# nchopin/particles

Measured on NVIDIA H100. Metric: particle-steps/sec (N x T), Bootstrap SV, higher is better.
Workload: dtype f64

## Files before the change

### particles_b200/csrc/smcb_filter.cu

```cuda
#include <stdlib.h>

#include "smcb_step.cuh"

extern template int bind_fk<GordonM>(smcb_filter *);
extern template int bind_fk<ThetaLogisticM>(smcb_filter *);
extern template int bind_fk<DiscreteCoxM>(smcb_filter *);
extern template int bind_fk<StochVolLevM>(smcb_filter *);
extern template int bind_fk<BearingsM>(smcb_filter *);
extern template int bind_fk<MvLinGaussM<2>>(smcb_filter *);
extern template int bind_fk<MvLinGaussM<3>>(smcb_filter *);
extern template int bind_fk<MvLinGaussM<4>>(smcb_filter *);

static int filter_bind(smcb_filter *f) {
    const smcb_filter_desc *d = &f->desc;
    bool bound = false;
    const int rc = with_model(d->model, d->dim, [&](auto m) {
        using M = decltype(m);
        if (M::D != d->dim) return SMCB_ENOSYS;
        bound = true;
        return bind_fk<M>(f);
    });
    if (bound) return rc;
    if (d->dim != 1 && d->model == SMCB_MODEL_BEARINGS) {
        set_error("fused BearingsOnly: state dimension must be 4");
        return SMCB_EINVAL;
    }
    if (d->dim == 1) set_error("fused filter: model id %d is not available in the fused 1-D family", d->model);
    else if (d->model == SMCB_MODEL_MVLINGAUSS) set_error("fused MVLinearGauss: dx must be 2, 3 or 4 (got %d)", d->dim);
    else set_error("fused filter: model id %d has no d-dimensional kernel", d->model);
    return SMCB_ENOSYS;
}

static int filter_setup(smcb_filter *f, smcb_ctx *c, const smcb_filter_desc *d);

extern "C" int smcb_filter_create(smcb_ctx *c, const smcb_filter_desc *d, smcb_filter **out) {
    SMCB_REQUIRE(c && d && out, "smcb_filter_create: NULL argument");
    SMCB_REQUIRE(d->n >= 1 && d->T >= 1, "smcb_filter_create: need n >= 1 and T >= 1");
    SMCB_REQUIRE(d->X[0] && d->X[1] && d->lw[0] && d->lw[1] && d->A && d->cdf && d->data && d->summaries,
                 "smcb_filter_create: NULL device buffer");
    SMCB_REQUIRE((d->index_offset & 1) == 0, "smcb_filter_create: index_offset must be even");
    SMCB_REQUIRE(d->dim >= 1 && d->dim <= 4, "smcb_filter_create: fused kernels exist for state dimension 1..4 (dim=%d)", d->dim);
    SMCB_REQUIRE(d->dy >= 1 && d->dy <= kMaxDy, "smcb_filter_create: observation dimension must be 1..%d", kMaxDy);
    SMCB_REQUIRE(d->essrmin >= 0.0 && d->essrmin <= 1.0, "smcb_filter_create: ESSrmin must be in [0, 1]");
    smcb_filter *f = new (std::nothrow) smcb_filter();
    SMCB_REQUIRE(f != nullptr, "smcb_filter_create: out of host memory");
    f->ctx = c;
    f->desc = *d;
    f->t_host = 0;
    f->timed = false;
    f->mem = nullptr;
    const int rc = filter_setup(f, c, d);
    if (rc) {
        if (f->mem) cudaFree(f->mem);
        delete f;
        return rc;
    }
    *out = f;
    return SMCB_OK;
}

static bool env_flag(const char *name, bool dflt) {
    const char *v = getenv(name);
    if (!v || !*v) return dflt;
    return v[0] != '0';
}

static int filter_setup(smcb_filter *f, smcb_ctx *c, const smcb_filter_desc *d) {
    int rc = filter_bind(f);
    if (rc) return rc;

    const int64_t n = d->n;
    FilterArgs &a = f->args;
    memset(&a, 0, sizeof(a));
    a.math_tab = c->math_tab;
    a.X[0] = d->X[0]; a.X[1] = d->X[1]; a.lw[0] = d->lw[0]; a.lw[1] = d->lw[1];
    a.A = reinterpret_cast<long long *>(d->A);
    a.cdf = d->cdf;
    a.su = (d->scheme == SMCB_RS_MULTINOMIAL) ? d->scratch : nullptr;
    SMCB_REQUIRE(d->scheme != SMCB_RS_MULTINOMIAL || d->scratch != nullptr,
                 "smcb_filter_create: multinomial needs desc.scratch of n + 2 doubles");
    a.data = d->data;
    a.sc = d->step_consts;
    a.summaries = d->summaries;
    a.moments = d->moments;
    a.z_in = d->z_in; a.u_in = d->u_in;
    a.dy = d->dy;
    a.n = n; a.n_global = d->n_global > 0 ? d->n_global : n;
    a.index_offset = d->index_offset; a.T = d->T;
    a.essrmin = d->essrmin;
    a.key = key_of(d->seed);
    {
        int dev = 0, sms = kSMs;
        SMCB_CUDA(cudaGetDevice(&dev));
        SMCB_CUDA(cudaDeviceGetAttribute(&sms, cudaDevAttrMultiProcessorCount, dev));
        const int64_t npairs = (n + 1) / 2;
        int64_t g = sms < kMaxStepGrid ? sms : kMaxStepGrid;
        const int64_t gmax = (npairs + f->block_size - 1) / f->block_size;
        if (g > gmax) g = gmax;
        if (g < 1) g = 1;
        int64_t chunk = (npairs + g - 1) / g;
        g = (npairs + chunk - 1) / chunk;
        a.chunk = chunk;
        f->grid_move = (int)g;
        a.grid = f->grid_move;
        const bool apf = d->fk == SMCB_FK_APF || d->fk == SMCB_FK_AUXBOOT;
        const bool mom = d->moments != nullptr;
        a.slab_lane = (!apf && !mom) ? 1 : 0;
        a.slab_stride = a.slab_lane ? 96 : 4 + (apf ? 4 : 0) + (mom ? 2 * d->dim : 0);
        const int64_t cap = f->slab_doubles / a.slab_stride;
        const int64_t n_iter = (chunk + f->pairs_per_iteration - 1) / f->pairs_per_iteration;
        int64_t slab_it = 2, n_small = 0;
        for (;; slab_it++) {
            const int64_t ns = (cap * slab_it - n_iter) / (slab_it - 1) - 1;
            const int64_t want = n_iter < 32 ? n_iter : 32;
            if (ns >= want) { n_small = ns < 0 ? 0 : (ns > n_iter / 8 ? n_iter / 8 : ns); break; }
        }
        if (n_small > n_iter) n_small = n_iter;
        a.slab_it = (int)slab_it;
        a.slab_small = (int)n_small;
    }
    a.world = d->world > 1 ? d->world : 1;
    a.rank = d->world > 1 ? d->rank : 0;
    {
        const char *v = getenv("SMCB_FUSE");
        const int mode = (!v || !*v) ? 1 : (v[0] == '0' ? 0 : (v[0] == '2' ? 2 : 1));
        a.fuse_mode = (d->dim == 1 && a.world == 1) ? mode : 0;
    }
    constexpr size_t kHdr = 512;
    static_assert(2 * sizeof(StepState) <= 256, "StepState outgrew its header slot");
    const size_t part = (size_t)kPartSlots * kMaxStepGrid * kPartStride * sizeof(double);
    const size_t agg = (size_t)(kMaxStepGrid + 8) * sizeof(double);
    const size_t slab = a.fuse_mode ? (size_t)f->grid_move * f->slab_doubles * sizeof(double) : 0;
    SMCB_CUDA(cudaMalloc(&f->mem, kHdr + part + agg + slab));
    SMCB_CUDA(cudaMemsetAsync(f->mem, 0, kHdr + part + agg, c->stream));
    a.st = reinterpret_cast<StepState *>(f->mem);
    a.fuse = reinterpret_cast<long long *>(f->mem + 256);
    a.bar = reinterpret_cast<unsigned long long *>(f->mem + 384);
    a.sync_timeout = reinterpret_cast<int *>(f->mem + 392);
    a.partials = reinterpret_cast<double *>(f->mem + kHdr);
    a.blk_agg = reinterpret_cast<double *>(f->mem + kHdr + part);
    a.fuse_slab = a.fuse_mode ? reinterpret_cast<double *>(f->mem + kHdr + part + agg) : nullptr;
    a.local_stats = d->local_stats;
    a.gathered = d->gathered;
    a.mail_local = (a.world > 1) ? d->mail_local : nullptr;
    for (int r = 0; r < 8; r++) a.mail_peer[r] = (a.world > 1 && r < a.world) ? d->mail_peer[r] : nullptr;
    SMCB_REQUIRE(a.world == 1 || (a.rank >= 0 && a.rank < a.world), "smcb_filter_create: bad rank");
    SMCB_REQUIRE(a.world == 1 || a.mail_local || (d->local_stats && d->gathered),
                 "smcb_filter_create: world > 1 needs either a peer mailbox or local_stats / gathered");
    SMCB_REQUIRE(a.world <= 8, "smcb_filter_create: at most 8 ranks");
    if (a.mail_local) {
        for (int r = 0; r < a.world; r++)
            SMCB_REQUIRE(a.mail_peer[r] != nullptr, "smcb_filter_create: mail_peer[%d] is NULL", r);
    }
    a.rs_global = (a.world > 1 && d->rs_global) ? 1 : 0;
    if (a.rs_global) {
        SMCB_REQUIRE(a.mail_local != nullptr, "smcb_filter_create: global resampling needs the peer mailbox");
        SMCB_REQUIRE((n & 1) == 0, "smcb_filter_create: global resampling needs an even shard size");
        if (d->scheme != SMCB_RS_SYSTEMATIC && d->scheme != SMCB_RS_STRATIFIED) {
            set_error("fused filter: global resampling over shards supports systematic and stratified");
            return SMCB_ENOSYS;
        }
        for (int r = 0; r < a.world; r++) {
            SMCB_REQUIRE(d->peer_X0[r] && d->peer_X1[r] && d->peer_cdf[r],
                         "smcb_filter_create: peer_X0 / peer_X1 / peer_cdf[%d] is NULL", r);
            a.pX[r][0] = d->peer_X0[r]; a.pX[r][1] = d->peer_X1[r]; a.pcdf[r] = d->peer_cdf[r];
        }
    }
    f->pdl = env_flag("SMCB_PDL", true);
    f->coop = env_flag("SMCB_COOP", false);
    return SMCB_OK;
}

extern "C" int smcb_filter_destroy(smcb_filter *f) {
    if (!f) return SMCB_OK;
    cudaStreamSynchronize(f->ctx->stream);
    cudaFree(f->mem);
    delete f;
    return SMCB_OK;
}

static int launch_one(smcb_filter *f) {
    if (f->t_host >= f->desc.T) {
        set_error("smcb_filter_step: all %lld steps already done (StopIteration)", (long long)f->desc.T);
        return SMCB_EINVAL;
    }
    int rc = (f->t_host == 0) ? f->launch_init(f) : f->launch_step(f);
    if (rc && f->t_host > 0 && (f->pdl || f->coop)) {
        cudaGetLastError();
        f->pdl = false; f->coop = false;
        rc = f->launch_step(f);
    }
    if (rc) return rc;
    f->t_host++;
    return SMCB_OK;
}

extern "C" int smcb_filter_step_local(smcb_filter *f) {
    SMCB_REQUIRE(f != nullptr && f->args.world > 1 && f->args.mail_local == nullptr,
                 "smcb_filter_step_local: not a sharded filter with the host-driven exchange");
    f->args.batch_end = f->t_host + 1;
    int rc = launch_one(f);
    if (rc) return rc;
    return f->launch_publish(f);
}

extern "C" int smcb_filter_step_finish(smcb_filter *f) {
    SMCB_REQUIRE(f != nullptr && f->args.world > 1, "smcb_filter_step_finish: not a sharded filter");
    return f->launch_tail(f);
}

extern "C" int smcb_filter_step(smcb_filter *f, int64_t nsteps) {
    SMCB_REQUIRE(f != nullptr, "smcb_filter_step: NULL filter");
    SMCB_REQUIRE(f->args.world == 1 || f->args.mail_local != nullptr,
                 "smcb_filter_step: sharded filters without a peer mailbox use step_local / step_finish");
    if (nsteps <= 0) return SMCB_OK;
    f->args.batch_end = f->t_host + nsteps;
    for (int64_t i = 0; i < nsteps; i++) {
        int rc = launch_one(f);
        if (rc) return rc;
    }
    return f->launch_tail(f);
}

extern "C" int smcb_filter_step_timed(smcb_filter *f, int64_t nsteps, double *out8) {
    SMCB_REQUIRE(f && out8, "smcb_filter_step_timed: NULL argument");
    SMCB_REQUIRE(nsteps >= 1 && nsteps <= 100000, "smcb_filter_step_timed: nsteps out of range");
    SMCB_REQUIRE(f->t_host + nsteps <= f->desc.T, "smcb_filter_step_timed: past the last step");
    SMCB_REQUIRE(f->args.world == 1, "smcb_filter_step_timed: single-device filters only");
    cudaStream_t s = f->ctx->stream;
    const size_t nev = (size_t)(nsteps + 1) * 2;
    cudaEvent_t *ev = new (std::nothrow) cudaEvent_t[nev];
    double *rows = new (std::nothrow) double[(size_t)nsteps * SMCB_SUMMARY_STRIDE];
    size_t made = 0;
    int rc = SMCB_OK;
    const int64_t t_first = f->t_host;
    auto fail = [&](cudaError_t e, const char *what) {
        set_error("smcb_filter_step_timed: %s -> %s", what, cudaGetErrorString(e));
        rc = SMCB_ECUDA;
    };
    if (!ev || !rows) { set_error("smcb_filter_step_timed: out of host memory"); rc = SMCB_EINVAL; }
    for (; rc == SMCB_OK && made < nev; made++) {
        cudaError_t e = cudaEventCreate(&ev[made]);
        if (e != cudaSuccess) { fail(e, "cudaEventCreate"); break; }
    }
    f->timed = true;
    f->args.batch_end = t_first + nsteps;
    for (int64_t i = 0; rc == SMCB_OK && i <= nsteps; i++) {
        cudaEventRecord(ev[2 * i], s);
        rc = (i < nsteps) ? launch_one(f) : f->launch_tail(f);
        cudaEventRecord(ev[2 * i + 1], s);
    }
    f->timed = false;
    if (rc == SMCB_OK) {
        cudaError_t e = cudaStreamSynchronize(s);
        if (e != cudaSuccess) fail(e, "cudaStreamSynchronize");
    }
    if (rc == SMCB_OK) {
        cudaError_t e = cudaMemcpy(rows, f->args.summaries + (size_t)t_first * SMCB_SUMMARY_STRIDE,
                                   sizeof(double) * nsteps * SMCB_SUMMARY_STRIDE, cudaMemcpyDeviceToHost);
        if (e != cudaSuccess) fail(e, "cudaMemcpy(summaries)");
    }
    if (rc == SMCB_OK) {
        for (int j = 0; j < 8; j++) out8[j] = 0.0;
        for (int64_t i = 0; i <= nsteps; i++) {
            float ms = 0.f;
            cudaEventElapsedTime(&ms, ev[2 * i], ev[2 * i + 1]);
            int kind = 2;
            if (i < nsteps) {
                const int64_t t = t_first + i;
                kind = (t == 0) ? 0 : (rows[(size_t)i * SMCB_SUMMARY_STRIDE + 2] != 0.0 ? 1 : 3);
            }
            out8[kind] += ms;
            out8[4 + kind] += 1.0;
        }
    }
    for (size_t i = 0; i < made; i++) cudaEventDestroy(ev[i]);
    delete[] ev;
    delete[] rows;
    return rc;
}
// ... 65 lines not shown
```

### particles_b200/csrc/smcb_step.cuh

```cuda
#pragma once
#include <string.h>

#include <new>
#include <type_traits>

#include "smcb_common.cuh"
#include "smcb_dispatch.cuh"
#include "smcb_math.cuh"
#include "smcb_models.cuh"
#include "smcb_scan.cuh"
#include "smcb_search.cuh"

using namespace smcb;

namespace smcb {

constexpr int kPartStride = 16;
constexpr int kMailStride = 32;
constexpr int kMailEpoch = 16;
constexpr int kMailScan = 17;
constexpr int kMaxStepGrid = 256;
constexpr int kMaxD = 4;
constexpr int kTailBlock = 256;
constexpr int kPartSlots = 4;
#ifndef SMCB_SPECULATE
#define SMCB_SPECULATE 1
#endif
template <class M> struct StepCfg {
    static constexpr int BS = 512;
    static constexpr int kU = (M::D == 1) ? 2 : 1;
    static constexpr int kStage = 8 * BS;
    static constexpr int kSlabRecords = 128;
    static constexpr int kSlabDoubles = kSlabRecords * 96;
    static constexpr size_t dyn_smem = kMathTabBytes + (size_t)(2 * kStage > kSlabDoubles ? 2 * kStage : kSlabDoubles) * sizeof(double);
};
constexpr int kScanGroupWarps = 2;
constexpr int kMovePairs = 2;

struct StepState {
    double logLt, log_mean_w, ess;
    double wm, ws, wq;
    long long t;
    long long nrs;
    int rs;
    int rs_next;
    int pad[2];
};

struct FilterArgs {
    double *X[2];
    double *lw[2];
    long long *A;
    double *cdf;
    double *su;
    const double *data;
    const double *sc;
    double *summaries;
    double *moments;
    const double *z_in, *u_in;
    StepState *st;
    int *sync_timeout;
    double *partials;
    int fuse_mode;
    int64_t batch_end;
    long long *fuse;
    double *fuse_slab;
    unsigned long long *bar;
    double *blk_agg;
    const double *math_tab;
    int slab_it;
    int slab_small;
    int slab_lane;
    int slab_stride;
    int64_t n, n_global, index_offset, T;
    int dy;
    int world, rank;
    int grid;
    int64_t chunk;
    double essrmin;
    Philox key;
    double *local_stats;
    const double *gathered;
    double *mail_local;
    double *mail_peer[8];
    int rs_global;
    const double *pX[8][2];
    const double *pcdf[8];
};

__device__ __forceinline__ void wait_epoch(const volatile double *flag, double epoch, int *timeout) {
    const long long t0 = clock64();
    if (*reinterpret_cast<volatile int *>(timeout)) return;
    while (*flag < epoch) {
        if (clock64() - t0 > 8000000000ll) { *timeout = 1; break; }
    }
    __threadfence_system();
}

__device__ __forceinline__ StepK step_consts(const FilterArgs &a, long long t) {
    StepK k;
    k.t = t;
#pragma unroll
    for (int i = 0; i < kMaxDy; i++) {
        k.yv[i] = (i < a.dy && t >= 0) ? a.data[t * a.dy + i] : 0.0;
        k.yn[i] = (i < a.dy && t + 1 < a.T) ? a.data[(t + 1) * a.dy + i] : 0.0;
    }
    k.y = k.yv[0];
    k.y_next = k.yn[0];
    k.sc0 = (a.sc && t >= 0) ? a.sc[t] : 0.0;
    return k;
}

__device__ __forceinline__ double fix_nan(double v) { return v != v ? -CUDART_INF : v; }

__device__ __forceinline__ void weights_scalars(const Lse3 &a, double n, double &log_mean, double &ess) {
    if (a.m == -CUDART_INF || a.m == CUDART_INF || a.m != a.m) {
        log_mean = CUDART_NAN;
        ess = CUDART_NAN;
        return;
    }
    log_mean = a.m + log(a.s / n);
    ess = (a.s * a.s) / a.q;
}

__device__ __forceinline__ double shift_factor(double m, double M) {
    return (m == -CUDART_INF) ? 0.0 : fexp_neg(m - M);
}

__device__ __forceinline__ double nanmax(double a, double b) { return (b > a || b != b) ? b : a; }

template <int NV, int BS, bool MAX>
__device__ __forceinline__ void block_reduce_all(double (&v)[NV], double *smem) {
    constexpr int NWARP = BS / 32;
    static_assert(NWARP <= 32, "one lane per warp in the second level");
    const int lane = threadIdx.x & 31, warp = threadIdx.x >> 5;
#pragma unroll
    for (int j = 0; j < NV; j++) {
#pragma unroll
        for (int mask = 16; mask > 0; mask >>= 1) {
            const double o = __shfl_xor_sync(0xffffffffu, v[j], mask);
            v[j] = MAX ? nanmax(v[j], o) : v[j] + o;
        }
    }
    if (lane == 0) {
#pragma unroll
        for (int j = 0; j < NV; j++) smem[warp * NV + j] = v[j];
    }
    __syncthreads();
    if (warp == 0) {
#pragma unroll
        for (int j = 0; j < NV; j++) {
            double x = (lane < NWARP) ? smem[lane * NV + j] : (MAX ? -CUDART_INF : 0.0);
#pragma unroll
            for (int mask = 16; mask > 0; mask >>= 1) {
                const double o = __shfl_xor_sync(0xffffffffu, x, mask);
                x = MAX ? nanmax(x, o) : x + o;
            }
            if (lane == 0) smem[NWARP * NV + j] = x;
        }
    }
    __syncthreads();
#pragma unroll
    for (int j = 0; j < NV; j++) v[j] = smem[NWARP * NV + j];
    __syncthreads();
}
template <int NV, int BS>
__device__ __forceinline__ void block_max_all(double (&v)[NV], double *smem) { block_reduce_all<NV, BS, true>(v, smem); }
template <int NV, int BS>
__device__ __forceinline__ void block_sum_all(double (&v)[NV], double *smem) { block_reduce_all<NV, BS, false>(v, smem); }

template <int D>
struct Acc {
    Lse3 w;
    double sx[D], sxx[D];
};

template <int D>
__device__ __forceinline__ void acc_init(Acc<D> &a) {
    a.w = lse3_empty();
#pragma unroll
    for (int c = 0; c < D; c++) { a.sx[c] = 0.0; a.sxx[c] = 0.0; }
}

template <int NV, int D, bool FINITE, bool MOM>
__device__ __forceinline__ void acc_add_batch_t(Acc<D> &a, const double (&v)[NV], const double (&x)[NV][D]) {
    double mb = v[0];
#pragma unroll
    for (int j = 1; j < NV; j++) mb = FINITE ? (v[j] > mb ? v[j] : mb) : fmax(mb, v[j]);
    if (mb > a.w.m) {
        const double r = texp_neg(a.w.m - mb);
        a.w.s *= r;
        a.w.q *= r * r;
        if (MOM) {
#pragma unroll
            for (int c = 0; c < D; c++) { a.sx[c] *= r; a.sxx[c] *= r; }
        }
        a.w.m = mb;
    }
    if (!FINITE && a.w.m == -CUDART_INF) return;
#pragma unroll
    for (int j = 0; j < NV; j++) {
        const double e = FINITE ? texp_sat(v[j] - a.w.m) : texp_neg(v[j] - a.w.m);
        a.w.s += e;
        a.w.q = fma(e, e, a.w.q);
        if (MOM && (FINITE || v[j] != -CUDART_INF)) {
#pragma unroll
            for (int c = 0; c < D; c++) {
                const double ex = e * x[j][c];
                a.sx[c] += ex;
                a.sxx[c] = fma(ex, x[j][c], a.sxx[c]);
            }
        }
    }
}
template <int NV, int D, bool FINITE = false>
__device__ __forceinline__ void acc_add_batch(Acc<D> &a, const double (&v)[NV], const double (&x)[NV][D], bool mom) {
    if (mom) acc_add_batch_t<NV, D, FINITE, true>(a, v, x);
    else acc_add_batch_t<NV, D, FINITE, false>(a, v, x);
}

struct StepSmem {
    double red[32 * 16];
    int next;
    double ringP[32];
    int ringF[32];
    double gwarp[16][8];
    double gpref[16][2];
    int gqn[16];
    long long gq[16][8][3];
    int *timeout_ptr;
    double peer[8][kMailStride];
    double goff[9], gpi[8];
    double pref[2];
    double carry[20];
};

__device__ __forceinline__ double shift_factor_t(double m, double M) {
    return (m == -CUDART_INF) ? 0.0 : texp_neg(m - M);
}

__device__ __forceinline__ double warp_max_nan(double v) {
#pragma unroll
    for (int mask = 16; mask > 0; mask >>= 1) {
        const double o = __shfl_xor_sync(0xffffffffu, v, mask);
        v = (o > v || o != o) ? o : v;
    }
    return v;
}
__device__ __forceinline__ double warp_sum(double v) {
#pragma unroll
    for (int mask = 16; mask > 0; mask >>= 1) v += __shfl_xor_sync(0xffffffffu, v, mask);
    return v;
}

template <int D, bool APF>
__device__ __forceinline__ void warp_reduce_to_slab(const Acc<D> &sa, const Lse3 &sx, bool mom, double *rec, int lane) {
    const double M = warp_max_nan(sa.w.m);
    const double e = shift_factor_t(sa.w.m, M);
    const double s = warp_sum(sa.w.s * e), q = warp_sum(sa.w.q * (e * e));
    if (lane == 0) { rec[0] = M; rec[1] = s; rec[2] = q; }
    int off = 4;
    if (APF) {
        const double Ma = warp_max_nan(sx.m);
        const double ea = shift_factor_t(sx.m, Ma);
        const double as_ = warp_sum(sx.s * ea), aq = warp_sum(sx.q * (ea * ea));
        if (lane == 0) { rec[4] = Ma; rec[5] = as_; rec[6] = aq; }
        off = 8;
    }
    if (mom) {
#pragma unroll
        for (int c = 0; c < D; c++) {
            const double a1 = warp_sum(sa.sx[c] * e), a2 = warp_sum(sa.sxx[c] * e);
            if (lane == 0) { rec[off + c] = a1; rec[off + D + c] = a2; }
        }
    }
}

template <int D, bool APF, int BS>
__device__ __forceinline__ void write_partial(const FilterArgs &a, long long t, const Acc<D> &acc, const Lse3 &aux,
                                              bool mom, StepSmem &sh, const double *s_slab = nullptr, int n_slab = 0) {
    const bool lane_rec = a.slab_lane != 0;
    const int n_rec = lane_rec ? n_slab * 32 : n_slab;
    auto rec_ptr = [&](int r) {
        return lane_rec ? s_slab + (size_t)(r >> 5) * a.slab_stride + (r & 31) : s_slab + (size_t)r * a.slab_stride;
    };
    const int rs_ = lane_rec ? 32 : 1;
    if (n_slab > 0) __syncthreads();
    double mx[2] = {acc.w.m, APF ? aux.m : -CUDART_INF};
    for (int r = threadIdx.x; r < n_rec; r += BS) {
        const double *rec = rec_ptr(r);
        mx[0] = nanmax(mx[0], rec[0]);
        if (APF && !lane_rec) mx[1] = nanmax(mx[1], rec[4]);
    }
    block_max_all<2, BS>(mx, sh.red);
    const double ew = shift_factor_t(acc.w.m, mx[0]);
    const double ea = APF ? shift_factor_t(aux.m, mx[1]) : 0.0;
    double v[4 + 2 * D];
    v[0] = acc.w.s * ew;
    v[1] = acc.w.q * (ew * ew);
    v[2] = APF ? aux.s * ea : 0.0;
    v[3] = APF ? aux.q * (ea * ea) : 0.0;
#pragma unroll
    for (int c = 0; c < D; c++) {
        v[4 + c] = mom ? acc.sx[c] * ew : 0.0;
        v[4 + D + c] = mom ? acc.sxx[c] * ew : 0.0;
    }
    for (int r = threadIdx.x; r < n_rec; r += BS) {
        const double *rec = rec_ptr(r);
        const double e = shift_factor_t(rec[0], mx[0]);
        v[0] += rec[rs_] * e;
        v[1] += rec[2 * rs_] * (e * e);
        if (!lane_rec) {
            if (APF) {
                const double e2 = shift_factor_t(rec[4], mx[1]);
                v[2] += rec[5] * e2;
                v[3] += rec[6] * (e2 * e2);
            }
            if (mom) {
                const int off = APF ? 8 : 4;
#pragma unroll
                for (int c = 0; c < D; c++) { v[4 + c] += rec[off + c] * e; v[4 + D + c] += rec[off + D + c] * e; }
            }
        }
    }
    if (mom) block_sum_all<4 + 2 * D, BS>(v, sh.red);
    else {
        double w4[4] = {v[0], v[1], v[2], v[3]};
        block_sum_all<4, BS>(w4, sh.red);
        v[0] = w4[0]; v[1] = w4[1]; v[2] = w4[2]; v[3] = w4[3];
    }
    if (threadIdx.x == 0) {
        double *p = a.partials + ((size_t)(t % kPartSlots) * kMaxStepGrid + blockIdx.x) * kPartStride;
        p[0] = mx[0]; p[1] = v[0]; p[2] = v[1]; p[3] = 0.0;
        p[4] = APF ? mx[1] : mx[0]; p[5] = APF ? v[2] : v[0]; p[6] = APF ? v[3] : v[1]; p[7] = 0.0;
#pragma unroll
        for (int c = 0; c < kMaxD; c++) {
            p[8 + c] = (c < D) ? v[4 + (c < D ? c : 0)] : 0.0;
            p[12 + c] = (c < D) ? v[4 + D + (c < D ? c : 0)] : 0.0;
        }
    }
}

__device__ __forceinline__ void merge16(double (&a)[16], const double *b) {
#pragma unroll
    for (int k = 0; k < 2; k++) {
        const double am = a[4 * k], bm = b[4 * k];
        const double M = (bm > am || bm != bm) ? bm : am;
        const double ea = shift_factor(am, M), eb = shift_factor(bm, M);
        a[4 * k] = M;
        a[4 * k + 1] = a[4 * k + 1] * ea + b[4 * k + 1] * eb;
        a[4 * k + 2] = a[4 * k + 2] * (ea * ea) + b[4 * k + 2] * (eb * eb);
        if (k == 0) {
#pragma unroll
            for (int c = 8; c < 16; c++) a[c] = a[c] * ea + b[c] * eb;
        }
    }
}

template <bool APF>
__device__ __forceinline__ void shard_totals(const FilterArgs &a, long long s, bool mom, StepSmem &sh, double (&loc)[16]) {
    const int G = a.grid, tid = threadIdx.x;
    if (tid < 32) {
        const double *base = a.partials + (size_t)(s % kPartSlots) * kMaxStepGrid * kPartStride;
        constexpr int kR = kMaxStepGrid / 32;
        double pm[kR], ps[kR], pq[kR], xm[kR], xs[kR], xq[kR];
        double mw = -CUDART_INF, ma = -CUDART_INF;
#pragma unroll
        for (int i = 0; i < kR; i++) {
            const int r = tid + 32 * i;
            pm[i] = -CUDART_INF; ps[i] = 0.0; pq[i] = 0.0; xm[i] = -CUDART_INF; xs[i] = 0.0; xq[i] = 0.0;
            if (r < G) {
                const double *row = base + (size_t)r * kPartStride;
                const double2 r0 = __ldcg(reinterpret_cast<const double2 *>(row));
                pm[i] = r0.x; ps[i] = r0.y; pq[i] = __ldcg(row + 2);
                if (APF) {
                    const double2 r1 = __ldcg(reinterpret_cast<const double2 *>(row + 4));
                    xm[i] = r1.x; xs[i] = r1.y; xq[i] = __ldcg(row + 6);
                }
            }
            mw = nanmax(mw, pm[i]);
            if (APF) ma = nanmax(ma, xm[i]);
        }
        mw = warp_max_nan(mw);
        if (APF) ma = warp_max_nan(ma);
        double v[12];
#pragma unroll
        for (int j2 = 0; j2 < 12; j2++) v[j2] = 0.0;
#pragma unroll
        for (int i = 0; i < kR; i++) {
            const int r = tid + 32 * i;
            const double ew = shift_factor(pm[i], mw);
            v[0] += ps[i] * ew;
            v[1] += pq[i] * (ew * ew);
            if (APF) {
                const double ea = shift_factor(xm[i], ma);
                v[2] += xs[i] * ea;
                v[3] += xq[i] * (ea * ea);
            }
            if (mom && r < G) {
                const double *row = base + (size_t)r * kPartStride + 8;
#pragma unroll
                for (int c = 0; c < 8; c++) v[4 + c] += __ldcg(row + c) * ew;
            }
        }
#pragma unroll
        for (int j2 = 0; j2 < 12; j2++)
            if (j2 < 4 || mom) v[j2] = warp_sum(v[j2]);
        if (tid == 0) {
            double *o = sh.peer[0];
            o[0] = mw; o[1] = v[0]; o[2] = v[1]; o[3] = 0.0;
            o[4] = APF ? ma : mw; o[5] = APF ? v[2] : v[0]; o[6] = APF ? v[3] : v[1]; o[7] = 0.0;
#pragma unroll
            for (int c = 0; c < 8; c++) o[8 + c] = v[4 + c];
        }
    }
    __syncthreads();
#pragma unroll
    for (int j2 = 0; j2 < 16; j2++) loc[j2] = sh.peer[0][j2];
    __syncthreads();
}

template <int BS>
__device__ __forceinline__ void cta_prefix(double v, StepSmem &sh, double &p_b, double &p_next) {
    const int tid = threadIdx.x, lane = tid & 31, warp = tid >> 5;
    const double iw = warp_scan_monotone(v, lane);
    if (lane == 31) sh.red[warp] = iw;
    __syncthreads();
    double woff = 0.0;
    for (int w_ = 0; w_ < BS / 32; w_++)
        if (w_ < warp) woff = woff + sh.red[w_];
    const double incl = woff + iw;
    if (tid == 0 && blockIdx.x == 0) sh.pref[0] = 0.0;
    if (tid + 1 == (int)blockIdx.x) sh.pref[0] = incl;
    if (tid == (int)blockIdx.x) sh.pref[1] = incl;
    __syncthreads();
    p_b = sh.pref[0];
    p_next = fmax(sh.pref[1], p_b);
    __syncthreads();
}

struct StepDecision {
    int rs;
    long long nrs_prev;
    double reset_c;
    double xm, xs;
    double p_b, p_next;
    double ess;
};

struct PrologueCarry {
    bool mom;
};

template <bool APF>
__device__ __forceinline__ bool prologue_begin(const FilterArgs &a, long long t, StepSmem &sh, bool writer,
                                               PrologueCarry &pc) {
    const long long s = t - 1;
    const int tid = threadIdx.x;
    pc.mom = writer && a.moments != nullptr;
    StepState prev;
// ... 1075 lines not shown
            su[0] = __ldcg(a.su + 2 * p) / zlast;
            su[1] = (2 * p + 1 < n) ? __ldcg(a.su + 2 * p + 1) / zlast : 2.0;
            if (2 * p == k0) s_su[0] = su[0];
            if (2 * p == k1) s_su[1] = su[0];
            if (2 * p + 1 == k1) s_su[1] = su[1];
        }
        __syncthreads();
        const double su_first = s_su[0], su_last = s_su[1];
        if (lo < 0) {
            lo = block_lower_bound<BS>(a.cdf, 0, n, su_first);
            lo = lo < n - 1 ? lo : n - 1;
            if (threadIdx.x == 0) issue(lo, buf);
            __syncthreads();
        }
        const int64_t sbase = lo & ~(int64_t)1;
        const int cnt = (int)((n - sbase) < kStage ? (n - sbase) : kStage);
        mbar_wait(&s_bar[buf], buf ? phase1 : phase0);
        if (buf) phase1 ^= 1u; else phase0 ^= 1u;
        const double *s_cdf = s_stage + (size_t)buf * kStage;
        const bool covered = (sbase + cnt >= n) || (s_cdf[cnt - 1] >= su_last);
        int64_t hi = lo;
        if (!covered) hi = block_lower_bound<BS>(a.cdf, lo, n, su_last);
        int64_t a0 = 0, a1 = 0;
        if (active) {
            if (covered) {
                int l0, l1;
                tile_search(s_cdf, (int)(lo - sbase), cnt, su[0], su[1], l0, l1);
                a0 = sbase + l0;
                a1 = sbase + l1;
                if (2 * p == k1) s_hi = a0;
                if (2 * p + 1 == k1) s_hi = a1;
            } else {
                const int64_t hi1 = hi < n ? hi + 1 : n;
                a0 = lower_bound_cg(a.cdf, lo, hi1, su[0]);
                a1 = lower_bound_cg(a.cdf, a0, hi1, su[1]);
            }
        }
        __syncthreads();
        const int64_t lo_next = covered ? (s_hi < n ? s_hi : n - 1) : (hi < n ? hi : n - 1);
        if (pbase + BS < pend && threadIdx.x == 0) issue(lo_next, buf ^ 1);
        if (active) {
            a0 = a0 < n - 1 ? a0 : n - 1;
            a1 = a1 < n - 1 ? a1 : n - 1;
            finish_pair<M, FK>(model, a, e, reset_c, acc, aux, p, Xi, Xi, a0, a1, a0, a1);
        }
        lo = lo_next;
        buf ^= 1;
    }
}

template <class M, int FK, int SCHEME>
__device__ __forceinline__ void move_global(const M &model, const FilterArgs &a, const StepEnv &e, double reset_c,
                                            double u_sys, const double *uin, Acc<M::D> &acc, Lse3 &aux, StepSmem &sh,
                                            double *s_stage, double *s_su, long long &s_hi) {
    constexpr int BS = StepCfg<M>::BS, kStage = StepCfg<M>::kStage;
    const long long t = e.io.t;
    const int cur = e.cur;
    const int64_t n = e.n, pstart = e.pstart, pend = e.pend;
    if (blockIdx.x == 0 && (int)threadIdx.x < a.world) {
        __threadfence_system();
        double *slot = a.mail_peer[threadIdx.x] + ((size_t)(t & 1) * a.world + a.rank) * kMailStride;
        *reinterpret_cast<volatile double *>(slot + kMailScan) = (double)(t + 1);
    }
    if ((int)threadIdx.x < a.world)
        wait_epoch(a.mail_local + ((size_t)(t & 1) * a.world + threadIdx.x) * kMailStride + kMailScan,
                   (double)(t + 1), a.sync_timeout);
    __syncthreads();
    const int world = a.world;
    const double M_ = (double)a.n_global;
    double *s_cdf = s_stage;
    int64_t lo = -1;
    int lo_shard = -1;
    for (int64_t pbase = pstart; pbase < pend; pbase += BS) {
        const int64_t p = pbase + threadIdx.x;
        const bool active = p < pend;
        const int64_t k0 = 2 * pbase;
        const int64_t ptop = pbase + BS < pend ? pbase + BS : pend;
        const int64_t k1 = 2 * ptop - 1;
        double su[2] = {2.0, 2.0};
        if (active) {
            const double g0 = (double)(a.index_offset + 2 * p);
            if (SCHEME == SMCB_RS_SYSTEMATIC) {
                su[0] = (u_sys + g0) / M_;
                su[1] = (u_sys + (g0 + 1.0)) / M_;
            } else {
                double u0, u1;
                if (uin) { u0 = uin[2 * p]; u1 = uin[2 * p + 1]; }
                else uniform_pair(a.key, (uint64_t)((a.index_offset >> 1) + p), (uint32_t)t, kPurposeUniform, u0, u1);
                su[0] = (u0 + g0) / M_;
                su[1] = (u1 + (g0 + 1.0)) / M_;
            }
            if (2 * p == k0) s_su[0] = su[0];
            if (2 * p + 1 == k1) s_su[1] = su[1];
        }
        __syncthreads();
        const double su_first = s_su[0], su_last = s_su[1];
        const int kf = shard_of(sh.goff, sh.gpi, world, su_first);
        const int kl = shard_of(sh.goff, sh.gpi, world, su_last);
        int ks[2] = {kf, kf};
        int64_t an[2] = {0, 0};
        if (kf == kl) {
            const double *cdf = a.pcdf[kf];
            const double off = sh.goff[kf], pi = sh.gpi[kf];
            const double v0 = fmin((su[0] - off) / pi, 1.0), v1 = fmin((su[1] - off) / pi, 1.0);
            const double v_first = fmin((su_first - off) / pi, 1.0), v_last = fmin((su_last - off) / pi, 1.0);
            if (lo < 0 || lo_shard != kf) lo = block_lower_bound<BS>(cdf, 0, n, v_first);
            if (lo > n - 1) lo = n - 1;
            lo_shard = kf;
            const int64_t sbase = lo & ~(int64_t)1;
            const int cnt = (int)((n - sbase) < kStage ? (n - sbase) : kStage);
            for (int i = 2 * threadIdx.x; i < cnt; i += 2 * BS) {
                if (i + 1 < cnt) *reinterpret_cast<double2 *>(&s_cdf[i]) = __ldcg(reinterpret_cast<const double2 *>(cdf + sbase + i));
                else s_cdf[i] = __ldcg(cdf + sbase + i);
            }
            __syncthreads();
            const bool covered = (sbase + cnt >= n) || (s_cdf[cnt - 1] >= v_last);
            int64_t hi = lo;
            if (!covered) hi = block_lower_bound<BS>(cdf, lo, n, v_last);
            if (active) {
                if (covered) {
                    int l0, l1;
                    tile_search(s_cdf, (int)(lo - sbase), cnt, v0, v1, l0, l1);
                    an[0] = sbase + l0;
                    an[1] = sbase + l1;
                    if (2 * p + 1 == k1) s_hi = an[1];
                } else {
                    const int64_t hi1 = hi < n ? hi + 1 : n;
                    an[0] = lower_bound_cg(cdf, lo, hi1, v0);
                    an[1] = lower_bound_cg(cdf, an[0], hi1, v1);
                }
            }
            __syncthreads();
            lo = covered ? (s_hi < n ? s_hi : n - 1) : (hi < n ? hi : n - 1);
        } else {
            if (active) {
#pragma unroll
                for (int j = 0; j < 2; j++) {
                    ks[j] = shard_of(sh.goff, sh.gpi, world, su[j]);
                    const double v = fmin((su[j] - sh.goff[ks[j]]) / sh.gpi[ks[j]], 1.0);
                    an[j] = lower_bound_cg(a.pcdf[ks[j]], 0, n, v);
                }
            }
            lo = -1;
        }
        if (active) {
            const int64_t a0 = an[0] < n - 1 ? an[0] : n - 1, a1 = an[1] < n - 1 ? an[1] : n - 1;
            finish_pair<M, FK>(model, a, e, reset_c, acc, aux, p, a.pX[ks[0]][cur], a.pX[ks[1]][cur], a0, a1,
                               (long long)ks[0] * n + a0, (long long)ks[1] * n + a1);
        }
        __syncthreads();
    }
}

template <class M, int FK, int SCHEME>
__global__ void __launch_bounds__(StepCfg<M>::BS, 1) k_step(M model, FilterArgs a, long long t) {
    constexpr bool APF = FkTraits<FK>::apf;
    constexpr int D = M::D, NZ = M::NZ, BS = StepCfg<M>::BS;
    extern __shared__ __align__(128) double s_dyn[];
    double *const s_stage = s_dyn + kMathTabDoubles;
    __shared__ StepSmem sh;
    __shared__ double s_su[2];
    __shared__ __align__(8) uint64_t s_bar[2];
    __shared__ __align__(8) uint64_t s_tabbar;
    __shared__ long long s_hi;
    __shared__ double s_warp[BS / 32];
    if (threadIdx.x == 0) { mtab_issue(a.math_tab, &s_tabbar); sh.next = 0; }
    cudaGridDependencySynchronize();
    cudaTriggerProgrammaticLaunchCompletion();
    PrologueCarry pc;
    const bool pred_rs = prologue_begin<APF>(a, t, sh, blockIdx.x == 0, pc);
    const bool speculate = SMCB_SPECULATE && a.world > 1 && a.mail_local != nullptr && !a.rs_global && !pred_rs;
    StepDecision dec;
    dec.rs = 0; dec.nrs_prev = 0; dec.reset_c = 0.0; dec.xm = 0.0; dec.xs = 1.0; dec.p_b = 0.0; dec.p_next = 0.0;
    dec.ess = 0.0;
    if (!speculate) dec = prologue_end<APF, BS>(a, t, sh, blockIdx.x == 0, true, pc);
    mbar_wait(&s_tabbar, 0);
    const int cur = (int)((t - 1) & 1);
    const bool rs = dec.rs != 0;
    if (a.fuse_mode != 0 && __ldcg(a.fuse) == t) {
        if (blockIdx.x == 0 && threadIdx.x == 0) a.fuse[rs ? 3 : 2] += 1;
        if (!rs) return;
    }
    bool fuse = false;
    if (D == 1 && !rs && a.fuse_mode != 0 && a.world == 1 && t + 1 < a.T && t + 1 < a.batch_end) {
        const double ess2 = (t >= 2) ? __ldcg(&a.st[(t - 2) & 1].ess) : dec.ess;
        fuse = a.fuse_mode == 2 || 2.0 * dec.ess - ess2 >= (double)a.n_global * a.essrmin;
    }
    if (fuse && blockIdx.x == 0 && threadIdx.x == 0) { a.fuse[0] = t + 1; a.fuse[1] += 1; }
    StepEnv e;
    e.io = step_io(a, t, NZ);
    e.kprev = step_consts(a, t - 1);
    e.cur = cur;
    e.n = a.n;
    e.vec_x = (D == 1) || ((a.n & 1) == 0);
    e.mom = a.moments != nullptr;
    cta_range(a, e.pstart, e.pend);

    Acc<D> acc;
    acc_init(acc);
    Lse3 aux = lse3_empty();
    int n_slab = 0;
    if (rs || stream_step<M, FK>(model, a, e, fuse, speculate, pc, dec, sh, s_stage, n_slab)) {
        const double *uin = a.u_in ? a.u_in + (size_t)t * (a.n + 1) : nullptr;
        const double u_sys = (SCHEME == SMCB_RS_SYSTEMATIC) ? systematic_u(a.key, t, uin) : 0.0;
        resample_scan<M, FK, SCHEME>(model, a, e, dec, u_sys, sh, s_stage, s_warp);
        if (SCHEME != SMCB_RS_MULTINOMIAL && !a.rs_global)
            move_counted<M, FK, SCHEME>(model, a, e, dec.reset_c, u_sys, uin, acc, aux);
        else if (SCHEME == SMCB_RS_MULTINOMIAL && !a.rs_global)
            move_tiles<M, FK>(model, a, e, dec.reset_c, acc, aux, s_stage, s_su, s_bar, s_hi);
        else
            move_global<M, FK, SCHEME>(model, a, e, dec.reset_c, u_sys, uin, acc, aux, sh, s_stage, s_su, s_hi);
    }
    write_partial<D, APF, BS>(a, t, acc, aux, e.mom, sh, s_stage, n_slab);
    if (fuse)
        write_partial<D, APF, BS>(a, t + 1, acc, aux, e.mom, sh, a.fuse_slab + (size_t)blockIdx.x * StepCfg<M>::kSlabDoubles,
                                  n_slab);
}

template <bool APF>
__global__ void __launch_bounds__(kTailBlock) k_tail(FilterArgs a, long long t) {
    __shared__ StepSmem sh;
    cudaGridDependencySynchronize();
    step_prologue<APF, kTailBlock>(a, t, sh, true, false);
}

template <bool APF>
__global__ void __launch_bounds__(kTailBlock) k_publish(FilterArgs a, long long s) {
    __shared__ StepSmem sh;
    double loc[16];
    shard_totals<APF>(a, s, true, sh, loc);
    if (threadIdx.x == 0)
        for (int i = 0; i < 16; i++) a.local_stats[i] = loc[i];
}

}

struct smcb_filter {
    smcb_ctx *ctx;
    smcb_filter_desc desc;
    FilterArgs args;
    char *mem;
    int grid_move;
    int block_size;
    size_t dyn_smem;
    int slab_doubles;
    int pairs_per_iteration;
    int64_t t_host;
    bool pdl, coop;
    bool timed;
    int (*launch_init)(smcb_filter *);
    int (*launch_step)(smcb_filter *);
    int (*launch_tail)(smcb_filter *);
    int (*launch_publish)(smcb_filter *);
};

template <class... Args>
static int launch_ex(smcb_filter *f, void (*kern)(Args...), int grid, int block, size_t smem, bool coop, bool pdl,
                     Args... args) {
    cudaLaunchConfig_t cfg = {};
    cfg.gridDim = dim3(grid);
    cfg.blockDim = dim3(block);
    cfg.dynamicSmemBytes = smem;
    cfg.stream = f->ctx->stream;
    cudaLaunchAttribute attr[2];
    int na = 0;
    if (coop) { attr[na].id = cudaLaunchAttributeCooperative; attr[na].val.cooperative = 1; na++; }
    if (pdl) {
        attr[na].id = cudaLaunchAttributeProgrammaticStreamSerialization;
        attr[na].val.programmaticStreamSerializationAllowed = 1;
        na++;
    }
    cfg.attrs = attr;
    cfg.numAttrs = na;
    SMCB_CUDA(cudaLaunchKernelEx(&cfg, kern, args...));
    f->ctx->launches++;
    return SMCB_OK;
}

template <class M, int FK, int SCHEME>
static int launch_step_t(smcb_filter *f) {
    M model;
    model.load(f->desc.params);
    return launch_ex(f, k_step<M, FK, SCHEME>, f->grid_move, f->block_size, f->dyn_smem, f->coop,
                     f->pdl && !f->timed, model, f->args, (long long)f->t_host);
}

template <class M, int FK>
static int launch_init_t(smcb_filter *f) {
    M model;
    model.load(f->desc.params);
    k_init<M, FK><<<f->grid_move, f->block_size, kMathTabBytes, f->ctx->stream>>>(model, f->args);
    f->ctx->launches++;
    SMCB_CUDA(cudaGetLastError());
    return SMCB_OK;
}

template <int FK>
static int launch_tail_t(smcb_filter *f) {
    return launch_ex(f, k_tail<FkTraits<FK>::apf>, 1, kTailBlock, 0, false, f->pdl && !f->timed, f->args,
                     (long long)f->t_host);
}

template <int FK>
static int launch_publish_t(smcb_filter *f) {
    k_publish<FkTraits<FK>::apf><<<1, kTailBlock, 0, f->ctx->stream>>>(f->args, (long long)(f->t_host - 1));
    f->ctx->launches++;
    SMCB_CUDA(cudaGetLastError());
    return SMCB_OK;
}

template <class M, int FK, int SCHEME>
static int bind_one(smcb_filter *f) {
    f->launch_init = launch_init_t<M, FK>;
    f->launch_step = launch_step_t<M, FK, SCHEME>;
    f->launch_tail = launch_tail_t<FK>;
    f->launch_publish = launch_publish_t<FK>;
    f->block_size = StepCfg<M>::BS;
    f->dyn_smem = StepCfg<M>::dyn_smem;
    f->slab_doubles = StepCfg<M>::kSlabDoubles;
    f->pairs_per_iteration = 32 * StepCfg<M>::kU;
    SMCB_CUDA(cudaFuncSetAttribute(k_step<M, FK, SCHEME>, cudaFuncAttributeMaxDynamicSharedMemorySize,
                                   (int)StepCfg<M>::dyn_smem));
    SMCB_CUDA(cudaFuncSetAttribute(k_init<M, FK>, cudaFuncAttributeMaxDynamicSharedMemorySize, (int)kMathTabBytes));
    int nb = 0;
    SMCB_CUDA(cudaOccupancyMaxActiveBlocksPerMultiprocessor(&nb, k_step<M, FK, SCHEME>, StepCfg<M>::BS,
                                                            StepCfg<M>::dyn_smem));
    if (nb < 1) {
        set_error("fused filter: the step kernel does not fit on an SM of this device");
        return SMCB_ECUDA;
    }
    return SMCB_OK;
}

template <class M, int FK>
static int bind_scheme(smcb_filter *f) {
    bool fused = false;
    const int rc = with_scheme(f->desc.scheme, [&](auto scheme) {
        fused = true;
        return bind_one<M, FK, decltype(scheme)::value>(f);
    });
    if (!fused)
        set_error("fused filter: resampling scheme %d is not fused (use systematic, stratified or "
                  "multinomial, or the unfused path)", f->desc.scheme);
    return rc;
}

template <class M>
int bind_fk(smcb_filter *f) {
    if (f->desc.fk < SMCB_FK_BOOTSTRAP || f->desc.fk > SMCB_FK_AUXBOOT) {
        set_error("fused filter: unknown Feynman-Kac kind %d", f->desc.fk);
        return SMCB_EINVAL;
    }
    bool offered = false;
    const int rc = with_fk<M>(f->desc.fk, [&](auto fk) {
        offered = true;
        return bind_scheme<M, decltype(fk)::value>(f);
    });
    if (offered) return rc;
    set_error("fused filter: model %d implements no proposal/logeta (Feynman-Kac kind %d)",
              f->desc.model, f->desc.fk);
    return SMCB_ENOSYS;
}
```

Baseline: 72.18 billion.

## Split 1-D step into streaming kernel and resample-only step kernel

For one-dimensional single-device filters, each step now launches a lean streaming kernel that handles non-resampling steps and exits early when resampling is needed. A second launch of k_step, specialised as RS_ONLY, returns immediately unless the previous step flagged resampling. The aim is to keep the common non-resampling path in a smaller kernel with less shared memory and fewer registers. The cost is a second launch every step, plus the branching and fallback logic that adds complexity and launch overhead.

After: 72.92 billion (median of 6 runs). 1.01x the previous value.

```diff
diff --git a/particles_b200/csrc/smcb_filter.cu b/particles_b200/csrc/smcb_filter.cu
--- a/particles_b200/csrc/smcb_filter.cu
+++ b/particles_b200/csrc/smcb_filter.cu
@@ -126,6 +126,7 @@
         const int mode = (!v || !*v) ? 1 : (v[0] == '0' ? 0 : (v[0] == '2' ? 2 : 1));
         a.fuse_mode = (d->dim == 1 && a.world == 1) ? mode : 0;
     }
+    f->split = d->dim == 1 && a.world == 1 && env_flag("SMCB_SPLIT", true);
     constexpr size_t kHdr = 512;
     static_assert(2 * sizeof(StepState) <= 256, "StepState outgrew its header slot");
     const size_t part = (size_t)kPartSlots * kMaxStepGrid * kPartStride * sizeof(double);
diff --git a/particles_b200/csrc/smcb_step.cuh b/particles_b200/csrc/smcb_step.cuh
--- a/particles_b200/csrc/smcb_step.cuh
+++ b/particles_b200/csrc/smcb_step.cuh
@@ -26,6 +26,9 @@
 #ifndef SMCB_SPECULATE
 #define SMCB_SPECULATE 1
 #endif
+#ifndef SMCB_STREAM_BS
+#define SMCB_STREAM_BS 512
+#endif
 template <class M> struct StepCfg {
     static constexpr int BS = 512;
     static constexpr int kU = (M::D == 1) ? 2 : 1;
@@ -33,6 +36,9 @@
     static constexpr int kSlabRecords = 128;
     static constexpr int kSlabDoubles = kSlabRecords * 96;
     static constexpr size_t dyn_smem = kMathTabBytes + (size_t)(2 * kStage > kSlabDoubles ? 2 * kStage : kSlabDoubles) * sizeof(double);
+    static constexpr int kStreamBS = SMCB_STREAM_BS;
+    static constexpr size_t stream_smem = kMathTabBytes + (size_t)kSlabDoubles * sizeof(double);
+    static_assert(kStreamBS >= BS && kStreamBS % 32 == 0, "k_stream reduces over the first BS threads");
 };
 constexpr int kScanGroupWarps = 2;
 constexpr int kMovePairs = 2;
@@ -142,7 +148,7 @@
             v[j] = MAX ? nanmax(v[j], o) : v[j] + o;
         }
     }
-    if (lane == 0) {
+    if (lane == 0 && warp < NWARP) {
 #pragma unroll
         for (int j = 0; j < NV; j++) smem[warp * NV + j] = v[j];
     }
@@ -285,9 +291,10 @@
         return lane_rec ? s_slab + (size_t)(r >> 5) * a.slab_stride + (r & 31) : s_slab + (size_t)r * a.slab_stride;
     };
     const int rs_ = lane_rec ? 32 : 1;
+    const int r0 = (int)threadIdx.x < BS ? (int)threadIdx.x : n_rec;
     if (n_slab > 0) __syncthreads();
     double mx[2] = {acc.w.m, APF ? aux.m : -CUDART_INF};
-    for (int r = threadIdx.x; r < n_rec; r += BS) {
+    for (int r = r0; r < n_rec; r += BS) {
         const double *rec = rec_ptr(r);
         mx[0] = nanmax(mx[0], rec[0]);
         if (APF && !lane_rec) mx[1] = nanmax(mx[1], rec[4]);
@@ -305,7 +312,7 @@
         v[4 + c] = mom ? acc.sx[c] * ew : 0.0;
         v[4 + D + c] = mom ? acc.sxx[c] * ew : 0.0;
     }
-    for (int r = threadIdx.x; r < n_rec; r += BS) {
+    for (int r = r0; r < n_rec; r += BS) {
         const double *rec = rec_ptr(r);
         const double e = shift_factor_t(rec[0], mx[0]);
         v[0] += rec[rs_] * e;
@@ -1687,10 +1694,39 @@
     }
 }
 
-template <class M, int FK, int SCHEME>
+__device__ __forceinline__ bool precomputed(const FilterArgs &a, long long t, bool rs) {
+    if (a.fuse_mode == 0 || __ldcg(a.fuse) != t) return false;
+    if (blockIdx.x == 0 && threadIdx.x == 0) a.fuse[rs ? 3 : 2] += 1;
+    return true;
+}
+
+template <int D>
+__device__ __forceinline__ bool fuse_next(const FilterArgs &a, long long t, const StepDecision &dec, bool rs) {
+    bool fuse = false;
+    if (D == 1 && !rs && a.fuse_mode != 0 && a.world == 1 && t + 1 < a.T && t + 1 < a.batch_end) {
+        const double ess2 = (t >= 2) ? __ldcg(&a.st[(t - 2) & 1].ess) : dec.ess;
+        fuse = a.fuse_mode == 2 || 2.0 * dec.ess - ess2 >= (double)a.n_global * a.essrmin;
+    }
+    if (fuse && blockIdx.x == 0 && threadIdx.x == 0) { a.fuse[0] = t + 1; a.fuse[1] += 1; }
+    return fuse;
+}
+
+__device__ __forceinline__ StepEnv step_env(const FilterArgs &a, long long t, int nz, int d) {
+    StepEnv e;
+    e.io = step_io(a, t, nz);
+    e.kprev = step_consts(a, t - 1);
+    e.cur = (int)((t - 1) & 1);
+    e.n = a.n;
+    e.vec_x = (d == 1) || ((a.n & 1) == 0);
+    e.mom = a.moments != nullptr;
+    cta_range(a, e.pstart, e.pend);
+    return e;
+}
+
+template <class M, int FK, int SCHEME, bool RS_ONLY>
 __global__ void __launch_bounds__(StepCfg<M>::BS, 1) k_step(M model, FilterArgs a, long long t) {
     constexpr bool APF = FkTraits<FK>::apf;
-    constexpr int D = M::D, NZ = M::NZ, BS = StepCfg<M>::BS;
+    constexpr int D = M::D, BS = StepCfg<M>::BS;
     extern __shared__ __align__(128) double s_dyn[];
     double *const s_stage = s_dyn + kMathTabDoubles;
     __shared__ StepSmem sh;
@@ -1699,9 +1735,14 @@
     __shared__ __align__(8) uint64_t s_tabbar;
     __shared__ long long s_hi;
     __shared__ double s_warp[BS / 32];
-    if (threadIdx.x == 0) { mtab_issue(a.math_tab, &s_tabbar); sh.next = 0; }
+    if (threadIdx.x == 0) { if (!RS_ONLY) mtab_issue(a.math_tab, &s_tabbar); sh.next = 0; }
     cudaGridDependencySynchronize();
     cudaTriggerProgrammaticLaunchCompletion();
+    if (RS_ONLY) {
+        const StepState *ps = a.st + ((t - 1) & 1);
+        if (__ldcg(&ps->t) != t - 1 || !__ldcg(&ps->rs_next)) return;
+        if (threadIdx.x == 0) mtab_issue(a.math_tab, &s_tabbar);
+    }
     PrologueCarry pc;
     const bool pred_rs = prologue_begin<APF>(a, t, sh, blockIdx.x == 0, pc);
     const bool speculate = SMCB_SPECULATE && a.world > 1 && a.mail_local != nullptr && !a.rs_global && !pred_rs;
@@ -1710,26 +1751,10 @@
     dec.ess = 0.0;
     if (!speculate) dec = prologue_end<APF, BS>(a, t, sh, blockIdx.x == 0, true, pc);
     mbar_wait(&s_tabbar, 0);
-    const int cur = (int)((t - 1) & 1);
-    const bool rs = dec.rs != 0;
-    if (a.fuse_mode != 0 && __ldcg(a.fuse) == t) {
-        if (blockIdx.x == 0 && threadIdx.x == 0) a.fuse[rs ? 3 : 2] += 1;
-        if (!rs) return;
-    }
-    bool fuse = false;
-    if (D == 1 && !rs && a.fuse_mode != 0 && a.world == 1 && t + 1 < a.T && t + 1 < a.batch_end) {
-        const double ess2 = (t >= 2) ? __ldcg(&a.st[(t - 2) & 1].ess) : dec.ess;
-        fuse = a.fuse_mode == 2 || 2.0 * dec.ess - ess2 >= (double)a.n_global * a.essrmin;
-    }
-    if (fuse && blockIdx.x == 0 && threadIdx.x == 0) { a.fuse[0] = t + 1; a.fuse[1] += 1; }
-    StepEnv e;
-    e.io = step_io(a, t, NZ);
-    e.kprev = step_consts(a, t - 1);
-    e.cur = cur;
-    e.n = a.n;
-    e.vec_x = (D == 1) || ((a.n & 1) == 0);
-    e.mom = a.moments != nullptr;
-    cta_range(a, e.pstart, e.pend);
+    const bool rs = RS_ONLY || dec.rs != 0;
+    if (!RS_ONLY && precomputed(a, t, rs) && !rs) return;
+    const bool fuse = !RS_ONLY && fuse_next<D>(a, t, dec, rs);
+    const StepEnv e = step_env(a, t, M::NZ, D);
 
     Acc<D> acc;
     acc_init(acc);
@@ -1752,6 +1777,35 @@
                                   n_slab);
 }
 
+template <class M, int FK>
+__global__ void __launch_bounds__(StepCfg<M>::kStreamBS, 1) k_stream(M model, FilterArgs a, long long t) {
+    static_assert(M::D == 1, "the d-dimensional filters run their streaming steps in k_step");
+    constexpr bool APF = FkTraits<FK>::apf;
+    constexpr int BS = StepCfg<M>::BS;
+    extern __shared__ __align__(128) double s_dyn[];
+    double *const s_stage = s_dyn + kMathTabDoubles;
+    __shared__ StepSmem sh;
+    __shared__ __align__(8) uint64_t s_tabbar;
+    if (threadIdx.x == 0) { mtab_issue(a.math_tab, &s_tabbar); sh.next = 0; }
+    cudaGridDependencySynchronize();
+    cudaTriggerProgrammaticLaunchCompletion();
+    const StepDecision dec = step_prologue<APF, BS>(a, t, sh, blockIdx.x == 0, false);
+    mbar_wait(&s_tabbar, 0);
+    const bool rs = dec.rs != 0;
+    if (precomputed(a, t, rs) || rs) return;
+    const bool fuse = fuse_next<1>(a, t, dec, rs);
+    const StepEnv e = step_env(a, t, M::NZ, 1);
+    const int n_slab = fuse ? stream_pass<M, FK, true>(model, a, e, sh, s_stage)
+                            : stream_pass<M, FK, false>(model, a, e, sh, s_stage);
+    Acc<1> acc;
+    acc_init(acc);
+    const Lse3 aux = lse3_empty();
+    write_partial<1, APF, BS>(a, t, acc, aux, e.mom, sh, s_stage, n_slab);
+    if (fuse)
+        write_partial<1, APF, BS>(a, t + 1, acc, aux, e.mom, sh, a.fuse_slab + (size_t)blockIdx.x * StepCfg<M>::kSlabDoubles,
+                                  n_slab);
+}
+
 template <bool APF>
 __global__ void __launch_bounds__(kTailBlock) k_tail(FilterArgs a, long long t) {
     __shared__ StepSmem sh;
@@ -1782,6 +1836,7 @@
     int pairs_per_iteration;
     int64_t t_host;
     bool pdl, coop;
+    bool split;
     bool timed;
     int (*launch_init)(smcb_filter *);
     int (*launch_step)(smcb_filter *);
@@ -1816,8 +1871,27 @@
 static int launch_step_t(smcb_filter *f) {
     M model;
     model.load(f->desc.params);
-    return launch_ex(f, k_step<M, FK, SCHEME>, f->grid_move, f->block_size, f->dyn_smem, f->coop,
-                     f->pdl && !f->timed, model, f->args, (long long)f->t_host);
+    const long long t = f->t_host;
+    if constexpr (M::D == 1) {
+        if (f->split) {
+            int rc = launch_ex(f, k_stream<M, FK>, f->grid_move, StepCfg<M>::kStreamBS, StepCfg<M>::stream_smem, false,
+                               f->pdl && !f->timed, model, f->args, t);
+            if (rc) return rc;
+            auto rs_step = [&] {
+                return launch_ex(f, k_step<M, FK, SCHEME, true>, f->grid_move, f->block_size, f->dyn_smem, f->coop,
+                                 f->pdl && !f->timed, model, f->args, t);
+            };
+            rc = rs_step();
+            if (rc && (f->pdl || f->coop)) {
+                cudaGetLastError();
+                f->pdl = false; f->coop = false;
+                rc = rs_step();
+            }
+            return rc;
+        }
+    }
+    return launch_ex(f, k_step<M, FK, SCHEME, false>, f->grid_move, f->block_size, f->dyn_smem, f->coop,
+                     f->pdl && !f->timed, model, f->args, t);
 }
 
 template <class M, int FK>
@@ -1854,12 +1928,25 @@
     f->dyn_smem = StepCfg<M>::dyn_smem;
     f->slab_doubles = StepCfg<M>::kSlabDoubles;
     f->pairs_per_iteration = 32 * StepCfg<M>::kU;
-    SMCB_CUDA(cudaFuncSetAttribute(k_step<M, FK, SCHEME>, cudaFuncAttributeMaxDynamicSharedMemorySize,
+    SMCB_CUDA(cudaFuncSetAttribute(k_step<M, FK, SCHEME, false>, cudaFuncAttributeMaxDynamicSharedMemorySize,
                                    (int)StepCfg<M>::dyn_smem));
     SMCB_CUDA(cudaFuncSetAttribute(k_init<M, FK>, cudaFuncAttributeMaxDynamicSharedMemorySize, (int)kMathTabBytes));
     int nb = 0;
-    SMCB_CUDA(cudaOccupancyMaxActiveBlocksPerMultiprocessor(&nb, k_step<M, FK, SCHEME>, StepCfg<M>::BS,
+    SMCB_CUDA(cudaOccupancyMaxActiveBlocksPerMultiprocessor(&nb, k_step<M, FK, SCHEME, false>, StepCfg<M>::BS,
                                                             StepCfg<M>::dyn_smem));
+    if constexpr (M::D == 1) {
+        SMCB_CUDA(cudaFuncSetAttribute(k_step<M, FK, SCHEME, true>, cudaFuncAttributeMaxDynamicSharedMemorySize,
+                                       (int)StepCfg<M>::dyn_smem));
+        SMCB_CUDA(cudaFuncSetAttribute(k_stream<M, FK>, cudaFuncAttributeMaxDynamicSharedMemorySize,
+                                       (int)StepCfg<M>::stream_smem));
+        int nb_rs = 0, nb_st = 0;
+        SMCB_CUDA(cudaOccupancyMaxActiveBlocksPerMultiprocessor(&nb_rs, k_step<M, FK, SCHEME, true>, StepCfg<M>::BS,
+                                                                StepCfg<M>::dyn_smem));
+        SMCB_CUDA(cudaOccupancyMaxActiveBlocksPerMultiprocessor(&nb_st, k_stream<M, FK>, StepCfg<M>::kStreamBS,
+                                                                StepCfg<M>::stream_smem));
+        nb = nb < nb_rs ? nb : nb_rs;
+        nb = nb < nb_st ? nb : nb_st;
+    }
     if (nb < 1) {
         set_error("fused filter: the step kernel does not fit on an SM of this device");
         return SMCB_ECUDA;
```
